# jmloveyj/ros_navigation

Measured on AMD Instinct MI355X. Metric: replan cycles/sec (HIMM+VFH++A*) on 4096x4096 grid, higher is better.
Workload: dtype int32; 1 GPU; full replan loop on 4096x4096 f32 grid (res 0.05 m); one step = one turn of the 20-stage A* pipeline = 20 passes of [100032-ray HIMM batch + fused compose -> 256 VFH+ poses -> 256 grid-A* queries (one launch)]; 30% rectangle obstacles (seed 2); 4 ray batches / pose sets / query sets in rotation; cycles_per_pass=256, rays_per_pass=100032, rotating_input_sets=4, astar_queries_checked=15360, astar_queries_answered=15360, astar_bucket_width=128000, astar_pipeline_depth=20, parallelism=query-sharded x1, full=False

## Files before the change

### ros_navigation_amd/csrc/astar_tile.hip

```cpp
#include "engine.hpp"
#include <algorithm>
#include <cstring>
#include <vector>

using namespace rna;

namespace rna {

constexpr int TI = 64, TJ = 16;
constexpr int TILE_WORDS = TI * TJ;
constexpr int AUX_WORDS = 64;
constexpr int MASK_STRIDE = TILE_WORDS + 32 + 128;
#ifndef RNA_TSA_WAVES
#define RNA_TSA_WAVES 8
#endif
#ifndef RNA_TSA_SUPER
#define RNA_TSA_SUPER 2
#endif
#ifndef RNA_TSA_HPASS
#define RNA_TSA_HPASS (RNA_TSA_SUPER == 2 ? 4 : (RNA_TSA_SUPER ? 8 : 16))
#endif
#ifndef RNA_TSA_FRESH
#define RNA_TSA_FRESH 0
#endif
#ifndef RNA_TSA_CONFIRM
#define RNA_TSA_CONFIRM 0
#endif
#ifndef RNA_TSA_IDLE_SLEEP
#define RNA_TSA_IDLE_SLEEP 4
#endif
#ifndef RNA_TSA_FIRST_ROWS
#define RNA_TSA_FIRST_ROWS 1
#endif
#ifndef RNA_TSA_REDBLACK
#define RNA_TSA_REDBLACK 1
#endif
#ifndef RNA_TSA_WAVES_PER_EU
#define RNA_TSA_WAVES_PER_EU 8
#endif
constexpr int TSA_WAVES = RNA_TSA_WAVES;
constexpr int TSA_MAX_TILE_WORDS = 2048;
constexpr int COST_S = 1000, COST_D = 1414;
constexpr int INF = 0x7fffffff;
constexpr int KU = 0x40000000;
constexpr int SCR_CNT = 84 + 192 + 48 + 64;
constexpr int SCR_WORDS = SCR_CNT + 4;
static_assert(SCR_WORDS % 4 == 0 && 276 % 4 == 0, "a wavefront's scratch starts on 16 bytes and so do the edge columns in it (ds_write_b128)");

__device__ __forceinline__ int tsa_octile(int i, int j, int gi, int gj) {
  const int dx = abs(i - gi), dy = abs(j - gj);
  const int mx = dx > dy ? dx : dy, mn = dx > dy ? dy : dx;
  return COST_S * mx + (COST_D - COST_S) * mn;
}
#ifndef RNA_TSA_SCOPE
#define RNA_TSA_SCOPE __HIP_MEMORY_SCOPE_AGENT
#endif
__device__ __forceinline__ unsigned ld_l2(const unsigned* p) {
  return __hip_atomic_load(p, __ATOMIC_RELAXED, RNA_TSA_SCOPE);
}
__device__ __forceinline__ int tsa_unwrap_lin(int lin, int rows, int cols, int s0, int s1) {
  int i = lin % rows - s0, j = lin / rows - s1;
  if (i < 0) i += rows;
  if (j < 0) j += cols;
  return j * rows + i;
}
__device__ __forceinline__ int tsa_buffer_lin(int lin, int rows, int cols, int s0, int s1) {
  int i = lin % rows + s0, j = lin / rows + s1;
  if (i >= rows) i -= rows;
  if (j >= cols) j -= cols;
  return j * rows + i;
}
__device__ __forceinline__ int lane_m1(int v) { return __builtin_amdgcn_update_dpp(0, v, 0x138, 0xF, 0xF, true); }
__device__ __forceinline__ int lane_p1(int v) { return __builtin_amdgcn_update_dpp(0, v, 0x130, 0xF, 0xF, true); }
// ... 27 lines not shown
#define TSA_OPEN(m, bit) ({ int r_; asm volatile("v_bfe_i32 %0, %1, %2, 1" : "=v"(r_) : "v"(m), "i"(bit)); r_; })
__device__ __forceinline__ int tsa_h24(int mx, int mn) {
  int a, r;
  asm("v_mul_u32_u24 %0, %2, %1" : "=v"(a) : "v"(mx), "s"(COST_S));
  asm("v_mad_u32_u24 %0, %1, %2, %3" : "=v"(r) : "v"(mn), "s"(COST_D - COST_S), "v"(a));
  return r;
}
__device__ __forceinline__ unsigned tsa_seed24(unsigned t, unsigned lane) {
  unsigned a, r;
  asm("v_mul_u32_u24 %0, %1, 29" : "=v"(a) : "v"(t));
  asm("v_mad_u32_u24 %0, %1, %2, %3" : "=v"(r) : "v"(lane), "s"(8191u), "v"(a));
  return r;
}
__device__ __forceinline__ int tsa_octile24(int i, int j, int gi, int gj) {
  const int dx = abs(i - gi), dy = abs(j - gj);
  return tsa_h24(max(dx, dy), min(dx, dy));
}
__device__ __forceinline__ int tsa_prop(int u, int h, int thr) { return (u - h >= thr) ? u : 0; }

__device__ __forceinline__ int tile_of(int i, int j, int tiles_i) { return (j >> 4) * tiles_i + (i >> 6); }
__device__ __forceinline__ int in_page(int i, int j) { return ((j & 15) << 6) + (i & 63); }
__device__ __forceinline__ int kdi_of(int k) { return (k == 0 || k == 3 || k == 5) ? -1 : ((k == 2 || k == 4 || k == 7) ? 1 : 0); }
__device__ __forceinline__ int kdj_of(int k) { return k < 3 ? -1 : (k > 4 ? 1 : 0); }

struct TsaStage {
  unsigned* pages;
  unsigned* paux;
  unsigned* tmap;
  unsigned* owner;
  int* nalloc;
  uint8_t* nbr_tm;
  int* perm;
  int* ticket;
  int cap;
};
__host__ __device__ inline size_t tsa_align256(size_t x) { return (x + 255) & ~(size_t)255; }
constexpr int TSA_COUNTER_WORDS = 16;
__host__ __device__ inline unsigned long long* tsa_counters_of(const TsaStage& S) {
  return reinterpret_cast<unsigned long long*>(reinterpret_cast<char*>(S.nalloc) - TSA_COUNTER_WORDS * sizeof(unsigned long long));
}

__global__ void __launch_bounds__(256) tsa_snapshot_kernel(const uint8_t* __restrict__ nbr, int rows, int cols, int tiles_i, int tiles_j,
                                                             uint8_t* __restrict__ nbr_tm, int s0, int s1) {
  __shared__ unsigned s_free[256];
  const int a = threadIdx.x & 63, bq = threadIdx.x >> 6;
  for (int t = blockIdx.x; t < tiles_i * tiles_j; t += gridDim.x) {
    const int i = (t % tiles_i) * TI + a, j0 = (t / tiles_i) * TJ + bq * 4;
    unsigned v = 0u;
    if (i < rows) {
      const int bi = i + s0 >= rows ? i + s0 - rows : i + s0;
#pragma unroll
      for (int k = 0; k < 4; ++k)
        if (j0 + k < cols) {
          const int bj = j0 + k + s1 >= cols ? j0 + k + s1 - cols : j0 + k + s1;
          v |= (unsigned)nbr[(size_t)bj * rows + bi] << (8 * k);
        }
    }
    uint8_t* out = nbr_tm + (size_t)t * MASK_STRIDE;
    reinterpret_cast<unsigned*>(out)[a * 4 + bq] = v;
    if (a == 0) reinterpret_cast<unsigned*>(out + TILE_WORDS)[bq] = v;
    if (a == TI - 1) reinterpret_cast<unsigned*>(out + TILE_WORDS + 16)[bq] = v;
    s_free[threadIdx.x] = (((v & 0xffu) != 0u) ? 1u : 0u) | (((v & 0xff00u) != 0u) ? 2u : 0u) | (((v & 0xff0000u) != 0u) ? 4u : 0u) |
                          (((v & 0xff000000u) != 0u) ? 8u : 0u);
    __syncthreads();
    if (bq == 0)
      reinterpret_cast<unsigned short*>(out + TILE_WORDS + 32)[a] =
// ... 772 lines not shown
  TSA_T(t_d);
  TSA_ACC(2, t_c, t_d);
  TSA_ACC(6, t_w0, t_d);
  if (lane_in == 0) { atomicAdd(&scr[SCR_CNT], (unsigned)__builtin_popcount(rowchg)); atomicAdd(&scr[SCR_CNT + 1], 1u); }
  }
tsa_job_done:
#ifndef RNA_TSA_UNSAFE_NOWAIT
  asm volatile("s_waitcnt vmcnt(0)" ::: "memory");
#endif
  {
    int t_f = t_in;
    asm volatile("" : "+s"(t_f));
    const int again = sch.finish(t_f, lane_in, spare, scr + SCR_CNT);
    if (!again) break;
    first_w = again >> 1;
    sticky_w = 1;
    TSA_CNT(7, 1);
    TSA_CNT(22, 1);
  }
  }
#undef TSA_ROW_CHANGED
#undef TSA_H
}

#ifndef RNA_TSA_NODES
#define RNA_TSA_NODES 3072
#endif
constexpr int TSA_NP = RNA_TSA_NODES;
constexpr int TSA_BMW = TSA_NP / 32;
#ifndef RNA_TSA_QC
#define RNA_TSA_QC 1024
#endif
constexpr int TSA_QC = RNA_TSA_QC;
constexpr unsigned POP_EMPTY = 0xffffffffu;
static_assert(TSA_NP % 32 == 0 && TSA_NP < 0xffff, "node indices are 16 bits, 0xffff = none");
static_assert(TSA_NP * 4 >= (TI + 2) * (TJ + 2) * 4 + TILE_WORDS, "the backtrace's LDS image lives in the queue memory");

__device__ __forceinline__ unsigned lds_ld(const unsigned* p) { return __hip_atomic_load(p, __ATOMIC_RELAXED, __HIP_MEMORY_SCOPE_WORKGROUP); }
__device__ __forceinline__ int lds_ldi(const int* p) { return __hip_atomic_load(p, __ATOMIC_RELAXED, __HIP_MEMORY_SCOPE_WORKGROUP); }

struct TsaLocalSched {
  int* best_;
  int* state_;
  unsigned* st2_;
  unsigned* far_;
  unsigned* node_;
  unsigned* head_;
  unsigned* bm_;
  unsigned* qc_;
  int* count_;
  int* spill_;
  unsigned* open_;
  int* open_left_;
  __device__ __forceinline__ int best() const { return __hip_atomic_load(best_, __ATOMIC_RELAXED, __HIP_MEMORY_SCOPE_WORKGROUP); }
  __device__ __forceinline__ void improve_best(int g) { atomicMin(best_, g); }
  __device__ __forceinline__ void overflow() { *state_ = 4; }
  __device__ __forceinline__ void pool_exhausted() { *state_ = 5; }
  __device__ __forceinline__ void act_far(int t) { atomicOr(&far_[t >> 5], 1u << (t & 31)); }
  __device__ __forceinline__ bool is_far(int t) const { return (lds_ld(&far_[t >> 5]) >> (t & 31)) & 1u; }
  __device__ __forceinline__ int node_alloc(unsigned seed) {
    unsigned w = ((seed & 0xffffu) * (unsigned)TSA_BMW) >> 16;
    for (int tries = 0; tries < 32; ++tries) {
      const unsigned v = lds_ld(&bm_[w]);
      if (v) {
        const unsigned b = v & (0u - v);
        if (atomicAnd(&bm_[w], ~b) & b) return (int)(w * 32u) + __builtin_ctz(b);
      } else {
        w = w + 1u == (unsigned)TSA_BMW ? 0u : w + 1u;
      }
    }
    return -1;
  }
  __device__ __forceinline__ void node_free(int idx) { atomicOr(&bm_[idx >> 5], 1u << (idx & 31)); }
  __device__ __forceinline__ void link(int idx, unsigned t, unsigned cls) {
    for (;;) {
      const unsigned hv = lds_ld(&head_[cls]);
      __hip_atomic_store(&node_[idx], (hv << 16) | t, __ATOMIC_RELAXED, __HIP_MEMORY_SCOPE_WORKGROUP);
      asm volatile("" ::: "memory");
      if (atomicCAS(&head_[cls], hv, ((hv + 0x10000u) & 0xffff0000u) | (unsigned)idx) == hv) break;
    }
  }
  __device__ __forceinline__ void push(unsigned t, unsigned cls, int lane, int* spare) {
    if (lane == 0) {
      const int idx = *spare >= 0 ? *spare : node_alloc(t * 29u);
      if (idx >= 0) {
        link(idx, t, cls);
        atomicAdd(count_, 1);
        __hip_atomic_store(&qc_[t & (unsigned)(TSA_QC - 1)], (t << 8) | cls, __ATOMIC_RELAXED, __HIP_MEMORY_SCOPE_WORKGROUP);
      } else {
        atomicOr(&far_[t >> 5], 1u << (t & 31));
        *spill_ = 1;
      }
    }
    *spare = -1;
  }
  __device__ __forceinline__ void wake8(bool w, int t, unsigned cls, int lane, int* spare) {
    const unsigned sh = 2u * ((unsigned)t & 15u);
    unsigned old = 2u;
    if (w) old = atomicOr(&st2_[t >> 4], 1u << sh) >> sh;
    bool q = w && !(old & 2u);
    const unsigned qi = (unsigned)t & (unsigned)(TSA_QC - 1);
    if (q && (old & 1u)) {
      const unsigned c = lds_ld(&qc_[qi]);
      if ((c >> 8) == (unsigned)t && (c & 0xffu) <= cls) q = false;
    }
    if (q) __hip_atomic_store(&qc_[qi], ((unsigned)t << 8) | cls, __ATOMIC_RELAXED, __HIP_MEMORY_SCOPE_WORKGROUP);
    const unsigned long long qm = __builtin_amdgcn_ballot_w64(q);
    if (!qm) return;
    const int reuse = *spare;
    *spare = -1;
    int idx = -1;
    if (q) {
      idx = (reuse >= 0 && lane == __builtin_ctzll(qm)) ? reuse : node_alloc(tsa_seed24((unsigned)t, (unsigned)lane));
      if (idx >= 0) {
        link(idx, (unsigned)t, cls);
      } else {
        atomicOr(&far_[t >> 5], 1u << (t & 31));
        *spill_ = 1;
      }
    }
    const unsigned long long okm = __builtin_amdgcn_ballot_w64(idx >= 0);
    if (okm && lane == __builtin_ctzll(okm)) atomicAdd(count_, __builtin_popcountll(okm));
  }
  __device__ __forceinline__ int finish(int t, int lane, int* spare, unsigned* cnt) {
    const unsigned sh = 2u * ((unsigned)t & 15u);
    int r = 0;
    if (lane == 0) {
      atomicAdd(&cnt[2], 1u);
#ifdef RNA_TSA_NO_STICKY
      if (false) {
#else
      if ((lds_ld(&st2_[t >> 4]) >> sh) & 1u) {
#endif
        atomicAnd(&st2_[t >> 4], ~(1u << sh));
// ... 139 lines not shown
      const unsigned mc = s_mask[il * 16 + jl];
      const unsigned un = s_tile[(jl + 1) * BW + il + 1 + off];
      const bool hit = (lane < 8) & (((mc >> k) & 1u) != 0u) & (un != 0u) & (un == uc + (unsigned)wk);
      const unsigned long long m = __ballot(hit);
      if (!m) { ok = false; break; }
      const int src = __builtin_ctz((unsigned)m);
      uc = (unsigned)__builtin_amdgcn_readlane((int)un, src);
      const int sdi = kdi_of(src), sdj = kdj_of(src);
      ci += sdi; cj += sdj; il += sdi; jl += sdj;
      if (il < 0 || jl < 0 || il >= TI || jl >= TJ) break;
    }
  }
#ifdef RNA_TSA_STATS
  if (lane == 0) { atomicAdd(&g_tsa_stat[27], bt_loads); atomicAdd(&g_tsa_stat[28], bt_load_ticks); atomicAdd(&g_tsa_stat[29], (unsigned long long)len); }
#endif
  if (!ok) {
    if (lane == 0) A.results[q] = rna_astar_result{1, 0, INF, r.expanded, r.rounds, r.buckets};
    return;
  }
  if (len > A.max_path_len || len > A.rev_cap) {
    if (lane == 0) A.results[q] = rna_astar_result{3, len, r.cost, r.expanded, r.rounds, r.buckets};
    return;
  }
  asm volatile("s_waitcnt vmcnt(0)" ::: "memory");
  __builtin_amdgcn_wave_barrier();
  int32_t* path = A.paths + (size_t)q * A.max_path_len;
  for (int i = lane; i < len; i += 64) path[i] = tsa_buffer_lin(rev[len - 1 - i], rows, cols, A.s0, A.s1);
  if (lane == 0) A.results[q] = rna_astar_result{0, len, r.cost, r.expanded, r.rounds, r.buckets};
}

template <int WAVES, bool RETRY>
__global__ void __launch_bounds__(WAVES * 64) __attribute__((amdgpu_waves_per_eu(RNA_TSA_WAVES_PER_EU, RNA_TSA_WAVES_PER_EU))) tsa_search_kernel(const TsaLaunch A) {
  constexpr int TSA_THREADS = WAVES * 64;
  __shared__ __attribute__((aligned(16))) unsigned s_scr[WAVES][SCR_WORDS];
  extern __shared__ unsigned s_dyn[];
  __shared__ __attribute__((aligned(16))) unsigned s_node[TSA_NP];
  __shared__ __attribute__((aligned(16))) unsigned s_head[TSA_NCLS];
  __shared__ unsigned s_bm[TSA_BMW];
  __shared__ unsigned s_qc[TSA_QC];
  __shared__ int s_best, s_state, s_bucket, s_bucket0, s_jobs_done, s_jobs_noop, s_jobs_sticky, s_expanded, s_nalloc, s_any;
  __shared__ int s_count, s_spill, s_idle, s_open_left, s_open_pos, s_reruns;

  __shared__ int s_q, s_rank;
  if (!RETRY) {
    if (threadIdx.x == 0) { const int k = atomicAdd(A.S.ticket, 1); s_rank = k; s_q = A.S.perm[k]; }
  } else {
    if (threadIdx.x == 0) { s_q = A.retry_list[A.retry_base + (int)blockIdx.x]; s_rank = 1 << 30; }
  }
  __syncthreads();
  const int q = __builtin_amdgcn_readfirstlane(s_q);
  if (q < 0) return;
  if (RETRY && threadIdx.x == 0) A.S2.ticket[8 + blockIdx.x] = q;
  const TsaStage& S = RETRY ? A.S2 : A.S;
  const int sl = RETRY ? (int)blockIdx.x : q;
#ifndef RNA_TSA_PRIO_FIRST
#define RNA_TSA_PRIO_FIRST 0
#endif
  if (__builtin_amdgcn_readfirstlane(s_rank) < A.prio_first) __builtin_amdgcn_s_setprio(3);
  const int tid = threadIdx.x, lane = tid & 63, wv = __builtin_amdgcn_readfirstlane(tid >> 6);
#ifdef RNA_TSA_STATS
  const unsigned long long t_kernel0 = wall_clock64();
#endif
  const int rows = A.rows, cols = A.cols, tiles_i = A.tiles_i, tiles_j = A.tiles_j;
  rna_astar_query qu = A.queries[q];
  const int ncell = rows * cols;
  const int ntile = tiles_i * tiles_j;
  const int nt_words = (ntile + 31) >> 5;
  unsigned* const s_st2 = s_dyn;
  unsigned* const s_open = s_dyn + 2 * nt_words;
  unsigned* const s_far = s_dyn + 3 * nt_words;
  rna_astar_result* const results = A.results;

  const bool valid = qu.start >= 0 && qu.goal >= 0 && qu.start < ncell && qu.goal < ncell;
  if (!valid) {
    if (tid == 0) results[q] = rna_astar_result{2, 0, INF, 0, 0, 0};
    return;
  }
  qu.start = tsa_unwrap_lin(qu.start, rows, cols, A.s0, A.s1);
  qu.goal = tsa_unwrap_lin(qu.goal, rows, cols, A.s0, A.s1);
  const int si = qu.start % rows, sj = qu.start / rows;
  const int gi = qu.goal % rows, gj = qu.goal / rows;

  TsaCtx C;
  C.rows = rows; C.cols = cols; C.tiles_i = tiles_i; C.tiles_j = tiles_j;
  C.tiles_magic = tiles_i > 1 ? (unsigned)(0x100000000ull / (unsigned)tiles_i) + 1u : 0u;
  C.pages = S.pages + (((size_t)sl * ((size_t)S.cap + 1)) << 10);
  C.paux = S.paux + (size_t)sl * ((size_t)S.cap + 1) * AUX_WORDS;
  C.tmap = S.tmap + (size_t)sl * ntile;
  C.owner = S.owner + (size_t)sl * (S.cap + 1);
  C.cap = S.cap;
  C.nalloc = &s_nalloc;
  C.nbr_tm = S.nbr_tm;
  C.gi = gi; C.gj = gj;
  C.ts = tile_of(si, sj, tiles_i); C.sa = si & (TI - 1); C.sb = sj & (TJ - 1);
  C.tg = tile_of(gi, gj, tiles_i); C.ga = gi & (TI - 1); C.gb = gj & (TJ - 1);

  for (int w = tid; w < 4 * nt_words; w += TSA_THREADS) s_dyn[w] = 0u;
  for (int w = tid; w < TSA_NCLS; w += TSA_THREADS) s_head[w] = 0xffffu;
  for (int w = tid; w < TSA_BMW; w += TSA_THREADS) s_bm[w] = 0xffffffffu;
  for (int w = tid; w < TSA_QC; w += TSA_THREADS) s_qc[w] = 0xffffffffu;
  if (lane >= 48) s_scr[wv][68 + lane - 48] = 0u;
  if (lane < 4) s_scr[wv][SCR_CNT + lane] = 0u;
  {
    const unsigned ms = C.nbr_tm[(size_t)C.ts * MASK_STRIDE + C.sa * 16 + C.sb], mg = C.nbr_tm[(size_t)C.tg * MASK_STRIDE + C.ga * 16 + C.gb];
    if (qu.goal != qu.start && (mg == 0u || ms == 0u)) {
      if (tid == 0) results[q] = rna_astar_result{1, 0, INF, 0, 0, 0};
      return;
    }
  }
  {
    const int used_raw = S.nalloc[sl];
    const int used = used_raw < C.cap ? used_raw : C.cap;
    if (used > 0) {
      uint4* pg4 = reinterpret_cast<uint4*>(C.pages + (1 << 10));
      for (size_t w = tid; w < (size_t)used * (TILE_WORDS / 4); w += TSA_THREADS) pg4[w] = make_uint4(0u, 0u, 0u, 0u);
      uint4* ax4 = reinterpret_cast<uint4*>(C.paux + AUX_WORDS);
      for (size_t w = tid; w < (size_t)used * (AUX_WORDS / 4); w += TSA_THREADS) ax4[w] = make_uint4(0u, 0u, 0u, 0u);
      for (int p = 1 + tid; p <= used; p += TSA_THREADS) C.tmap[C.owner[p]] = 0u;
      asm volatile("s_waitcnt vmcnt(0)" ::: "memory");
    }
  }
  int key_shift = 0;
  while (((long long)A.bucket_width >> key_shift) > TSA_NCLS - 1) ++key_shift;
  if (tid == 0) {
    s_best = INF; s_state = 0; s_jobs_done = 0; s_jobs_noop = 0; s_jobs_sticky = 0; s_expanded = 0; s_nalloc = 0;
    s_bucket = tsa_octile(si, sj, gi, gj) / A.bucket_width;
    s_bucket0 = s_bucket;
    s_spill = 0; s_idle = 0; s_open_pos = 0; s_reruns = 0;
    s_count = 1; s_open_left = 1;
  }
  __syncthreads();
  if (tid == 0) s_open[C.ts >> 5] = 1u << (C.ts & 31);
  __syncthreads();

#ifdef RNA_TSA_STATS
  unsigned long long tsa_acc[24] = {};
  const unsigned long long t_life0 = wall_clock64();
  const unsigned long long c_life0 = __builtin_amdgcn_s_memtime();
#endif
#ifdef RNA_TSA_IDLE
  unsigned long long idle_ticks = 0ull;
  const unsigned long long t_wave0 = __builtin_amdgcn_s_memtime();
#endif
  TsaLocalSched sch{&s_best, &s_state, s_st2, s_far, s_node, s_head, s_bm, s_qc, &s_count, &s_spill, s_open, &s_open_left};
  int spare = -1;

  for (;;) {
    const int bucket = __builtin_amdgcn_readfirstlane(lds_ldi(&s_bucket));
    const long long bucket_end = ((long long)bucket + 1) * A.bucket_width;
    const unsigned bucket_end_u = bucket_end > 0x80000000LL ? 0x80000000u : (unsigned)bucket_end;
    const long long key_base_ll = (long long)KU - (long long)bucket * A.bucket_width;
    const int key_base = key_base_ll < -(long long)INF ? -INF : (int)key_base_ll;
    bool idle = false;
    bool open_blocked = false;
#ifdef RNA_TSA_IDLE
    unsigned long long t_idle0 = 0ull;
#endif
    for (;;) {
      TSA_T(t_p0);
      if (lds_ldi(&s_state) >= 4) break;
      if (idle) {
        if (lds_ldi(&s_idle) == WAVES) break;
        if (lds_ldi(&s_count) <= 0) { __builtin_amdgcn_s_sleep(RNA_TSA_IDLE_SLEEP); continue; }
        if (lane == 0) atomicSub(&s_idle, 1);
        idle = false;
#ifdef RNA_TSA_IDLE
        idle_ticks += __builtin_amdgcn_s_memtime() - t_idle0;
#endif
      }
      int t = -1;
      int first = 0;
      const int open_left = lds_ldi(&s_open_left);
      if (!open_blocked && open_left > 0) {
        const int pos = lds_ldi(&s_open_pos);
        const unsigned w = pos + lane < nt_words ? lds_ld(&s_open[pos + lane]) : 0u;
        const unsigned long long nz = __builtin_amdgcn_ballot_w64(w != 0u);
        if (!nz) {
          if (lane == 0) atomicCAS(&s_open_pos, pos, pos + 64 >= nt_words ? 0 : pos + 64);
          continue;
        }
        const int l0 = __builtin_ctzll(nz);
        const unsigned w0 = (unsigned)__builtin_amdgcn_readlane((int)w, l0);
        const int b0 = __builtin_ctz(w0);
        const int tt = ((pos + l0) << 5) + b0;
        const unsigned sh = 2u * ((unsigned)tt & 15u);
        int r = 0;
        if (lane == 0) {
          if ((atomicAnd(&s_open[pos + l0], ~(1u << b0)) >> b0) & 1u) {
            const unsigned old = atomicOr(&s_st2[tt >> 4], 2u << sh) >> sh;
            if (old & 2u) {
              atomicOr(&s_open[pos + l0], 1u << b0);
              atomicOr(&s_st2[tt >> 4], 1u << sh);
              r = 2;
            } else {
              atomicAnd(&s_st2[tt >> 4], ~(1u << sh));
              atomicSub(&s_open_left, 1);
              atomicSub(&s_count, 1);
              r = 1;
            }
          }
        }
        r = __builtin_amdgcn_readfirstlane(r);
        if (r == 0) continue;
        if (r == 2) { open_blocked = true; continue; }
        t = tt;
        first = 1;
      } else {
        open_blocked = false;
        const unsigned e = sch.pop(lane, &spare);
        if (e == POP_EMPTY) {
          if (open_left > 0) { __builtin_amdgcn_s_sleep(2); continue; }
          if (lane == 0) atomicAdd(&s_idle, 1);
          idle = true;
#ifdef RNA_TSA_IDLE
          t_idle0 = __builtin_amdgcn_s_memtime();
#endif
          continue;
        }
        const int tt = (int)(e & 0xffffu);
        const unsigned sh = 2u * ((unsigned)tt & 15u);
        int r = 0;
        if (lane == 0) {
          unsigned w = lds_ld(&s_st2[tt >> 4]);
          while (((w >> sh) & 3u) == 1u) {
            const unsigned got = atomicCAS(&s_st2[tt >> 4], w, (w | (2u << sh)) & ~(1u << sh));
            if (got == w) { r = 1; break; }
            w = got;
          }
          if (r == 1 && open_left > 0 && ((atomicAnd(&s_open[tt >> 5], ~(1u << (tt & 31))) >> (tt & 31)) & 1u)) {
            atomicSub(&s_open_left, 1);
            atomicSub(&s_count, 1);
            r = 2;
          }
        }
        r = __builtin_amdgcn_readfirstlane(r);
        if (r <= 0) continue;
        t = tt;
        first = r >> 1;
      }
#ifdef RNA_TSA_TAKE_SLEEP
      __builtin_amdgcn_s_sleep(RNA_TSA_TAKE_SLEEP);
#endif
      TSA_T(t_p1);
      TSA_ACC(4, t_p0, t_p1);
      TSA_CNT(7, 1);
#if defined(RNA_TSA_JOBPRIO)
      __builtin_amdgcn_s_setprio(RNA_TSA_JOBPRIO);
#endif
      tsa_job(sch, s_scr[wv], lane, t, C, first, bucket_end_u, key_base, key_shift, &spare TSA_ACC_ARG);
#if defined(RNA_TSA_JOBPRIO)
      __builtin_amdgcn_s_setprio(RNA_TSA_IDLEPRIO);
#endif
    }
    __syncthreads();
#ifdef RNA_TSA_IDLE
    if (idle) idle_ticks += __builtin_amdgcn_s_memtime() - t_idle0;
#endif
    if (s_state >= 4) break;
    int tid_r = threadIdx.x;
    asm volatile("" : "+v"(tid_r));
    const bool spilled = s_spill != 0;
    __syncthreads();
    if (tid_r == 0) {
      if (!spilled && s_best != INF && (long long)s_best < bucket_end) s_state = 1;
      if (spilled) s_reruns += 1;
      s_any = 0; s_spill = 0; s_idle = 0; s_open_pos = 0;
    }
    __syncthreads();
    if (s_state == 1) break;
    int cnt = 0;
    for (int w = tid_r; w < nt_words; w += TSA_THREADS) {
      const unsigned b = s_far[w];
      s_open[w] = b;
      s_far[w] = 0u;
      cnt += __popc(b);
    }
    if (cnt) atomicAdd(&s_any, cnt);
    __syncthreads();
    if (tid_r == 0) {
      if (!s_any) s_state = (s_best != INF) ? 1 : 2;
      else { s_count = s_any; s_open_left = s_any; if (!spilled) s_bucket += 1; }
    }
    __syncthreads();
    if (s_state != 0) break;
  }
#ifdef RNA_TSA_IDLE
  if (lane == 0) {
    atomicAdd(&tsa_counters_of(S)[8], __builtin_amdgcn_s_memtime() - t_wave0);
    atomicAdd(&tsa_counters_of(S)[9], idle_ticks);
  }
#endif
  if (lane == 0) {
    atomicAdd(&s_expanded, (int)s_scr[wv][SCR_CNT] * TI);
    atomicAdd(&s_jobs_done, (int)s_scr[wv][SCR_CNT + 2]);
    atomicAdd(&s_jobs_noop, (int)(s_scr[wv][SCR_CNT + 2] - s_scr[wv][SCR_CNT + 1]));
    atomicAdd(&s_jobs_sticky, (int)s_scr[wv][SCR_CNT + 3]);
  }
  __syncthreads();
  if (tid == 0) {
    unsigned long long* const cnt = tsa_counters_of(S);
    atomicAdd(&cnt[0], 1ull);
    atomicAdd(&cnt[1], (unsigned long long)s_nalloc);
    atomicAdd(&cnt[2], (unsigned long long)s_jobs_done);
    atomicAdd(&cnt[3], (unsigned long long)s_jobs_noop);
    atomicAdd(&cnt[4], (unsigned long long)s_jobs_sticky);
    atomicAdd(&cnt[5], (unsigned long long)(s_expanded / TI));
    atomicAdd(&cnt[6], (unsigned long long)(s_bucket - s_bucket0 + 1));
    if (s_reruns) atomicAdd(&cnt[7], (unsigned long long)s_reruns);
  }
#ifdef RNA_TSA_STATS
// ... 41 lines not shown
    for (int r = 0; r < TSA_RETRY; ++r)
      if (served[r] == q) { sl = r; retried = true; }
  if (!retried)
    for (int r = 0; r < n_retried; ++r)
      if (retry_list[r] == q) { if (threadIdx.x == 0) counts[q] = -1; return; }
  const TsaStage& S = retried ? S_retry : S_main;
  if (threadIdx.x == 0) s_cnt = 0;
  __syncthreads();
  const rna_astar_result r = results[q];
  int cnt = 0;
  if (r.status == 0 || r.status == 3) {
    const int goal = tsa_unwrap_lin(queries[q].goal, rows, cols, s0, s1);
    const int gi = goal % rows, gj = goal / rows;
    const int used = S.nalloc[sl];
    for (size_t w = threadIdx.x; w < ((size_t)used << 10); w += blockDim.x) {
      const int p = 1 + (int)(w >> 10), l = (int)(w & 1023);
      const int t = (int)S.owner[(size_t)sl * (S.cap + 1) + p];
      const int i = (t % tiles_i) * TI + (l & (TI - 1)), j = (t / tiles_i) * TJ + (l >> 6);
      const unsigned u = S.pages[(((size_t)sl * ((size_t)S.cap + 1) + p) << 10) + l];
      if (u != 0u && i < rows && j < cols && (KU - (int)u) + tsa_octile(i, j, gi, gj) <= r.cost) ++cnt;
    }
  }
  atomicAdd(&s_cnt, cnt);
  __syncthreads();
  if (threadIdx.x == 0) counts[q] = s_cnt;
}

static inline int tsa_ntile(const rna_engine* e) {
  return ((e->geom.size[0] + TI - 1) / TI) * ((e->geom.size[1] + TJ - 1) / TJ);
}
bool tsa_supported(const rna_engine* e) { return (size_t)tsa_ntile(e) <= (size_t)TSA_MAX_TILE_WORDS * 32; }
int tsa_tiles(const rna_engine* e) { return tsa_ntile(e); }
size_t tsa_pool_bytes(int max_queries, int cap) { return (size_t)max_queries * ((size_t)cap + 1) * (TILE_WORDS + AUX_WORDS) * sizeof(unsigned); }
size_t tsa_aux_bytes(const rna_engine* e, int max_queries, int cap) {
  const size_t ntile = (size_t)tsa_ntile(e);
  return 256 + 2 * tsa_align256((size_t)max_queries * sizeof(int)) + tsa_align256(ntile * MASK_STRIDE) +
         tsa_align256((size_t)max_queries * ntile * sizeof(unsigned)) + tsa_align256((size_t)max_queries * ((size_t)cap + 1) * sizeof(unsigned));
}
static TsaStage tsa_stage_view(const rna_engine* e, int slot) {
  const AstarDevice& a = e->astar;
  const size_t ntile = (size_t)tsa_ntile(e);
  char* base = static_cast<char*>(a.tsa_aux[slot]);
  TsaStage S;
  S.cap = a.page_cap;
  S.pages = reinterpret_cast<unsigned*>(a.g[slot]);
  S.paux = S.pages + (((size_t)a.max_queries * ((size_t)S.cap + 1)) << 10);
  S.ticket = reinterpret_cast<int*>(base);
  base += 256;
  S.nalloc = reinterpret_cast<int*>(base);
  base += tsa_align256((size_t)a.max_queries * sizeof(int));
  S.perm = reinterpret_cast<int*>(base);
  base += tsa_align256((size_t)a.max_queries * sizeof(int));
  S.nbr_tm = reinterpret_cast<uint8_t*>(base);
  base += tsa_align256(ntile * MASK_STRIDE);
  S.tmap = reinterpret_cast<unsigned*>(base);
  base += tsa_align256((size_t)a.max_queries * ntile * sizeof(unsigned));
  S.owner = reinterpret_cast<unsigned*>(base);
  return S;
}
size_t tsa_retry_pool_bytes(const rna_engine* e) { return tsa_pool_bytes(TSA_RETRY, tsa_ntile(e)); }
size_t tsa_retry_aux_bytes(const rna_engine* e) {
  const size_t ntile = (size_t)tsa_ntile(e);
  return 256 + tsa_align256(TSA_RETRY * sizeof(int)) + tsa_align256((size_t)TSA_RETRY * ntile * sizeof(unsigned)) +
         tsa_align256((size_t)TSA_RETRY * (ntile + 1) * sizeof(unsigned)) + tsa_align256((size_t)e->astar.max_queries * sizeof(int));
}
static int* tsa_retry_list(const rna_engine* e, int slot) {
  const size_t ntile = (size_t)tsa_ntile(e);
  return reinterpret_cast<int*>(static_cast<char*>(e->astar.tsa_aux_retry[slot]) + 256 + tsa_align256(TSA_RETRY * sizeof(int)) +
                                tsa_align256((size_t)TSA_RETRY * ntile * sizeof(unsigned)) + tsa_align256((size_t)TSA_RETRY * (ntile + 1) * sizeof(unsigned)));
}
static int* tsa_retry_served(const rna_engine* e, int slot) { return reinterpret_cast<int*>(e->astar.tsa_aux_retry[slot]) + 8; }
static int* tsa_retry_count(const rna_engine* e, int slot) { return tsa_retry_served(e, slot) + TSA_RETRY; }
static TsaStage tsa_retry_view(const rna_engine* e, int slot, const TsaStage& main) {
  const AstarDevice& a = e->astar;
  const size_t ntile = (size_t)tsa_ntile(e);
  char* base = static_cast<char*>(a.tsa_aux_retry[slot]);
  TsaStage S = main;
  S.cap = (int)ntile;
  S.pages = reinterpret_cast<unsigned*>(a.g_retry[slot]);
  S.paux = S.pages + (((size_t)TSA_RETRY * ((size_t)S.cap + 1)) << 10);
  S.ticket = reinterpret_cast<int*>(base);
  base += 256;
  S.nalloc = reinterpret_cast<int*>(base);
  base += tsa_align256(TSA_RETRY * sizeof(int));
  S.tmap = reinterpret_cast<unsigned*>(base);
  base += tsa_align256((size_t)TSA_RETRY * ntile * sizeof(unsigned));
  S.owner = reinterpret_cast<unsigned*>(base);
  return S;
}
int tsa_retry_prepare(rna_engine* e, int slot) {
  hipLaunchKernelGGL(tsa_fill_pages_kernel, dim3(2048), dim3(256), 0, e->stream, reinterpret_cast<uint4*>(e->astar.g_retry[slot]),
                     tsa_retry_pool_bytes(e) / sizeof(uint4));
  RNA_HIP(e, hipGetLastError());
  return RNA_OK;
}
int tsa_stage_prepare(rna_engine* e, int slot) {
  const TsaStage S = tsa_stage_view(e, slot);
  const size_t pages = (size_t)e->astar.max_queries * ((size_t)S.cap + 1);
  hipLaunchKernelGGL(tsa_fill_pages_kernel, dim3(8192), dim3(256), 0, e->stream, reinterpret_cast<uint4*>(S.pages),
                     pages * (TILE_WORDS + AUX_WORDS) / 4);
  RNA_HIP(e, hipGetLastError());
  return RNA_OK;
}

size_t tsa_ring_bytes(const rna_engine* e, int max_queries) {
  return 256 + tsa_align256((size_t)max_queries * sizeof(int)) + tsa_align256((size_t)tsa_ntile(e) * MASK_STRIDE);
}
static_assert(sizeof(TsaLaunch) <= sizeof(AstarDevice::last_launch[0]), "AstarDevice::last_launch holds a TsaLaunch");

int tsa_retry_launch(rna_engine* e, int slot, hipStream_t search_stream, int count) {
  AstarDevice& a = e->astar;
  TsaLaunch A;
  memcpy(&A, a.last_launch[slot], sizeof(A));
  A.retry = 1;
  A.retry_count = nullptr;
  A.S2 = tsa_retry_view(e, slot, A.S);
  for (int base = 0; base < count; base += TSA_RETRY) {
    A.retry_base = base;
    const int wgs = std::min(TSA_RETRY, count - base);
    if (a.depth > 1) hipLaunchKernelGGL((tsa_search_kernel<TSA_WAVES, true>), dim3(wgs), dim3(TSA_WAVES * 64), a.last_lds[slot], search_stream, A);
    else hipLaunchKernelGGL((tsa_search_kernel<16, true>), dim3(wgs), dim3(16 * 64), a.last_lds[slot], search_stream, A);
    RNA_HIP(e, hipGetLastError());
  }
  return RNA_OK;
}

int tsa_launch(rna_engine* e, int slot, hipStream_t init_stream, hipStream_t search_stream, hipEvent_t ev_init,
               const rna_astar_query* q_dev, int n, int32_t* paths_dev, int max_len, rna_astar_result* res_dev) {
  AstarDevice& a = e->astar;
  const int rows = e->geom.size[0], cols = e->geom.size[1];
  const int ti = (rows + TI - 1) / TI, tj = (cols + TJ - 1) / TJ;
  TsaStage S = tsa_stage_view(e, slot);
  hipStream_t prep_stream = search_stream;
  int ring = -1;
  if (ev_init) {
    ring = (int)(a.launches % (unsigned long long)a.ring_n);
    char* base = a.ring_mem + (size_t)ring * a.ring_stride;
    S.ticket = reinterpret_cast<int*>(base);
    S.perm = reinterpret_cast<int*>(base + 256);
    S.nbr_tm = reinterpret_cast<uint8_t*>(base + 256 + tsa_align256((size_t)a.max_queries * sizeof(int)));
    { const int rc = side_stream(e, &prep_stream); if (rc != RNA_OK) return rc; }
    RNA_HIP(e, hipEventRecord(ev_init, init_stream));
    RNA_HIP(e, hipStreamWaitEvent(prep_stream, ev_init, 0));
    if (a.ring_used[ring]) RNA_HIP(e, hipStreamWaitEvent(prep_stream, a.ring_free[ring], 0));
  }
  {
    KernelTimer kt(e, RNA_K_ASTAR_INIT, prep_stream);
    hipLaunchKernelGGL(tsa_snapshot_kernel, dim3(std::min(ti * tj, 4096)), dim3(256), 0, prep_stream, e->nbr, rows, cols, ti, tj, S.nbr_tm,
                       e->geom.start[0], e->geom.start[1]);
    RNA_HIP(e, hipGetLastError());
  }
  if (ev_init) {
    RNA_HIP(e, hipEventRecord(a.snap_done[slot], prep_stream));
    a.snap_pending[slot] = true;
  }
  {
    KernelTimer kt(e, RNA_K_ASTAR_RESET, prep_stream);
    const int ranked = n <= 2048 ? 1 : 0;
    hipLaunchKernelGGL(tsa_prepare_kernel, dim3(1), dim3(256), ranked ? (size_t)n * sizeof(int) : 0, prep_stream, S, q_dev, n, rows, cols, ranked,
                       a.g_retry[slot] ? tsa_retry_served(e, slot) : nullptr);
    RNA_HIP(e, hipGetLastError());
  }
  if (ev_init) {
    RNA_HIP(e, hipEventRecord(a.ev_prep, prep_stream));
    RNA_HIP(e, hipStreamWaitEvent(search_stream, a.ev_prep, 0));
  }
  {
    KernelTimer kt(e, RNA_K_ASTAR_SEARCH, search_stream);
    const size_t nt_bytes = (size_t)((ti * tj + 31) / 32) * sizeof(unsigned);
    TsaLaunch A;
    memset(&A, 0, sizeof(A));
    A.rows = rows; A.cols = cols; A.tiles_i = ti; A.tiles_j = tj; A.s0 = e->geom.start[0]; A.s1 = e->geom.start[1];
    A.queries = q_dev; A.S = S; A.bucket_width = a.bucket_width; A.paths = paths_dev; A.max_path_len = max_len;
    A.rev_all = a.rev[slot]; A.rev_cap = a.rev_cap; A.results = res_dev;
    A.retry = 0; A.n = n; A.S2 = S;
    A.prio_first = a.depth > 1 ? RNA_TSA_PRIO_FIRST : 0;
    if (const char* pf = getenv("RNA_TSA_PRIO_FIRST")) A.prio_first = atoi(pf);
    size_t lds_dyn = 4 * nt_bytes;
    if (const char* pad = getenv("RNA_TSA_LDS_PAD")) lds_dyn += (size_t)atoi(pad);
    const bool can_retry = a.g_retry[slot] != nullptr && a.retry_flag != nullptr;
    A.retry_count = can_retry ? tsa_retry_count(e, slot) : nullptr;
    A.retry_list = can_retry ? tsa_retry_list(e, slot) : nullptr;
    A.retry_base = 0;
    if (can_retry) a.retry_flag[slot] = 0;
    a.last_retried[slot] = 0;
    static const bool wide_env = getenv("RNA_TSA_WIDE") != nullptr;
    const bool wide = wide_env || n <= 32;
    if (a.depth > 1 && !wide) hipLaunchKernelGGL((tsa_search_kernel<TSA_WAVES, false>), dim3(n), dim3(TSA_WAVES * 64), lds_dyn, search_stream, A);
    else hipLaunchKernelGGL((tsa_search_kernel<16, false>), dim3(n), dim3(16 * 64), lds_dyn, search_stream, A);
    RNA_HIP(e, hipGetLastError());
    memcpy(a.last_launch[slot], &A, sizeof(A));
    a.last_lds[slot] = lds_dyn;
    a.retry_armed[slot] = A.retry_count != nullptr;
    if (A.retry_count) RNA_HIP(e, hipMemcpyAsync(a.retry_flag + slot, A.retry_count, sizeof(int), hipMemcpyDeviceToHost, search_stream));
  }
  if (ring >= 0) {
    RNA_HIP(e, hipEventRecord(a.ring_free[ring], search_stream));
    a.ring_used[ring] = true;
  }
  return RNA_OK;
}

int tsa_counters_read(rna_engine* e, unsigned long long* out, bool reset) {
  AstarDevice& a = e->astar;
  for (int k = 0; k < TSA_COUNTER_WORDS; ++k) out[k] = 0ull;
  for (int d = 0; d < AstarDevice::MAX_DEPTH; ++d) {
    for (int view = 0; view < 2; ++view) {
      char* base = static_cast<char*>(view ? a.tsa_aux_retry[d] : a.tsa_aux[d]);
      if (!base) continue;
      unsigned long long w[TSA_COUNTER_WORDS];
      char* cnt = base + 256 - sizeof(w);
      RNA_HIP(e, hipMemcpyAsync(w, cnt, sizeof(w), hipMemcpyDeviceToHost, e->stream));
      if (reset) RNA_HIP(e, hipMemsetAsync(cnt, 0, sizeof(w), e->stream));
      RNA_HIP(e, hipStreamSynchronize(e->stream));
      for (int k = 0; k < TSA_COUNTER_WORDS; ++k) out[k] += w[k];
    }
  }
  return RNA_OK;
}

#ifdef RNA_TSA_STATS
void tsa_stats_dump() {
  unsigned long long st[32];
  if (hipMemcpyFromSymbol(st, HIP_SYMBOL(g_tsa_stat), sizeof(st)) != hipSuccess) return;
  const double jobs = (double)st[7];
// ... 38 lines not shown
```

### ros_navigation_amd/csrc/engine.hpp

```cpp
#pragma once

#include <hip/hip_runtime.h>

#include <cstdint>
#include <cstdio>
#include <string>
#include <vector>

#include "../../include/rna.h"
#include "gridmath.hpp"

namespace rna {

constexpr int TILE = 64;

struct HimmSlot { int cell; int head; int len; int offset; };

struct HimmScratch {
  int cap_rays = 0;
  int n_slots = 0;
  rna_ray* rays_dev = nullptr;
  int4* desc = nullptr;
  int* ncells = nullptr;
  int* next = nullptr;
// ... 37 lines not shown
#ifndef RNA_ASTAR_MAX_DEPTH
#define RNA_ASTAR_MAX_DEPTH 20
#endif
  static constexpr int MAX_DEPTH = RNA_ASTAR_MAX_DEPTH;
  int depth = 4;
  int32_t* g[MAX_DEPTH] = {};
  int2* queues[MAX_DEPTH] = {};
  int32_t* rev[MAX_DEPTH] = {};
  int rev_cap = 16800;
  int mode = 1;
  int page_cap = 0;
  int page_cap_request = 0;
  void* tsa_aux[MAX_DEPTH] = {};
  int32_t* g_retry[MAX_DEPTH] = {};
  void* tsa_aux_retry[MAX_DEPTH] = {};
  hipStream_t side[MAX_DEPTH] = {};
  hipEvent_t done[MAX_DEPTH] = {};
  hipEvent_t snap_done[MAX_DEPTH] = {};
  bool snap_pending[MAX_DEPTH] = {};
  bool busy[MAX_DEPTH] = {};
  unsigned long long stage_seq[MAX_DEPTH] = {};
  hipEvent_t ev_init = nullptr;
  static constexpr int MAX_RING = 2 * MAX_DEPTH;
  int ring_n = 0;
  char* ring_mem = nullptr;
  size_t ring_stride = 0;
  hipEvent_t ring_free[MAX_RING] = {};
  bool ring_used[MAX_RING] = {};
  hipEvent_t ev_prep = nullptr;
  int* retry_flag = nullptr;
  bool retry_armed[MAX_DEPTH] = {};
  int last_retried[MAX_DEPTH] = {};
  size_t last_lds[MAX_DEPTH] = {};
  alignas(8) unsigned char last_launch[MAX_DEPTH][384] = {};
  unsigned long long launches = 0;
  int last_slot = 0;
  size_t field_stride = 0;
  rna_astar_query* queries_dev = nullptr;
  rna_astar_result* results_dev = nullptr;
  int32_t* paths_dev = nullptr;
  int paths_cap = 0;
  const rna_astar_query* last_queries = nullptr;
  const rna_astar_result* last_results = nullptr;
  int last_n = 0;
};

struct FootprintPlan {
  double r = 0.0, res = 0.0, mag = 0.0;
  int R = 0;
  int K = 0;
  int band = 0;
  int n_ties = 0;
  int w[64] = {};
};

struct ProfSlot {
  double total_ms = 0;
  int64_t launches = 0;
  std::vector<std::pair<hipEvent_t, hipEvent_t>> pending;
};

}

struct rna_engine {
  rna::Geom geom{};
  int device = 0;
// ... 124 lines not shown
```

Measured before the change: 164,100 replan cycles/s.

## Move open/far tile bitmaps from LDS to global and allow 4-wave search kernel

Moves the per-query open and far tile bitsets out of dynamic LDS into a per-slot global buffer that is accessed with agent-scope atomics, which halves the dynamic LDS footprint. Templates the local scheduler on the queue-cache size so that a 4-wave variant can use a smaller LDS cache. Adds a runtime env selection between 4 and 8 waves and records the chosen width for retry launches. The aim is lower LDS usage per workgroup and higher occupancy, at the cost of global-memory latency and extra atomics on the bitmap operations in the hot scheduling loop.

```diff
diff --git a/ros_navigation_amd/csrc/astar_tile.hip b/ros_navigation_amd/csrc/astar_tile.hip
--- a/ros_navigation_amd/csrc/astar_tile.hip
+++ b/ros_navigation_amd/csrc/astar_tile.hip
@@ -39,6 +39,7 @@
 #define RNA_TSA_WAVES_PER_EU 8
 #endif
 constexpr int TSA_WAVES = RNA_TSA_WAVES;
+static_assert(TSA_WAVES == 4 || TSA_WAVES == 8, "the pipelined search kernel is instantiated for 4 and 8 wavefronts");
 constexpr int TSA_MAX_TILE_WORDS = 2048;
 constexpr int COST_S = 1000, COST_D = 1414;
 constexpr int INF = 0x7fffffff;
@@ -132,6 +133,7 @@
   uint8_t* nbr_tm;
   int* perm;
   int* ticket;
+  unsigned* tbits;
   int cap;
 };
 __host__ __device__ inline size_t tsa_align256(size_t x) { return (x + 255) & ~(size_t)255; }
@@ -970,6 +972,7 @@
 #define RNA_TSA_QC 1024
 #endif
 constexpr int TSA_QC = RNA_TSA_QC;
+constexpr int TSA_QC_NARROW = 256;
 constexpr unsigned POP_EMPTY = 0xffffffffu;
 static_assert(TSA_NP % 32 == 0 && TSA_NP < 0xffff, "node indices are 16 bits, 0xffff = none");
 static_assert(TSA_NP * 4 >= (TI + 2) * (TJ + 2) * 4 + TILE_WORDS, "the backtrace's LDS image lives in the queue memory");
@@ -977,6 +980,7 @@
 __device__ __forceinline__ unsigned lds_ld(const unsigned* p) { return __hip_atomic_load(p, __ATOMIC_RELAXED, __HIP_MEMORY_SCOPE_WORKGROUP); }
 __device__ __forceinline__ int lds_ldi(const int* p) { return __hip_atomic_load(p, __ATOMIC_RELAXED, __HIP_MEMORY_SCOPE_WORKGROUP); }
 
+template <int QC>
 struct TsaLocalSched {
   int* best_;
   int* state_;
@@ -995,7 +999,7 @@
   __device__ __forceinline__ void overflow() { *state_ = 4; }
   __device__ __forceinline__ void pool_exhausted() { *state_ = 5; }
   __device__ __forceinline__ void act_far(int t) { atomicOr(&far_[t >> 5], 1u << (t & 31)); }
-  __device__ __forceinline__ bool is_far(int t) const { return (lds_ld(&far_[t >> 5]) >> (t & 31)) & 1u; }
+  __device__ __forceinline__ bool is_far(int t) const { return (ld_l2(&far_[t >> 5]) >> (t & 31)) & 1u; }
   __device__ __forceinline__ int node_alloc(unsigned seed) {
     unsigned w = ((seed & 0xffffu) * (unsigned)TSA_BMW) >> 16;
     for (int tries = 0; tries < 32; ++tries) {
@@ -1024,7 +1028,7 @@
       if (idx >= 0) {
         link(idx, t, cls);
         atomicAdd(count_, 1);
-        __hip_atomic_store(&qc_[t & (unsigned)(TSA_QC - 1)], (t << 8) | cls, __ATOMIC_RELAXED, __HIP_MEMORY_SCOPE_WORKGROUP);
+        __hip_atomic_store(&qc_[t & (unsigned)(QC - 1)], (t << 8) | cls, __ATOMIC_RELAXED, __HIP_MEMORY_SCOPE_WORKGROUP);
       } else {
         atomicOr(&far_[t >> 5], 1u << (t & 31));
         *spill_ = 1;
@@ -1037,7 +1041,7 @@
     unsigned old = 2u;
     if (w) old = atomicOr(&st2_[t >> 4], 1u << sh) >> sh;
     bool q = w && !(old & 2u);
-    const unsigned qi = (unsigned)t & (unsigned)(TSA_QC - 1);
+    const unsigned qi = (unsigned)t & (unsigned)(QC - 1);
     if (q && (old & 1u)) {
       const unsigned c = lds_ld(&qc_[qi]);
       if ((c >> 8) == (unsigned)t && (c & 0xffu) <= cls) q = false;
@@ -1243,12 +1247,13 @@
 template <int WAVES, bool RETRY>
 __global__ void __launch_bounds__(WAVES * 64) __attribute__((amdgpu_waves_per_eu(RNA_TSA_WAVES_PER_EU, RNA_TSA_WAVES_PER_EU))) tsa_search_kernel(const TsaLaunch A) {
   constexpr int TSA_THREADS = WAVES * 64;
+  constexpr int QC = WAVES == 4 ? TSA_QC_NARROW : TSA_QC;
   __shared__ __attribute__((aligned(16))) unsigned s_scr[WAVES][SCR_WORDS];
   extern __shared__ unsigned s_dyn[];
   __shared__ __attribute__((aligned(16))) unsigned s_node[TSA_NP];
   __shared__ __attribute__((aligned(16))) unsigned s_head[TSA_NCLS];
   __shared__ unsigned s_bm[TSA_BMW];
-  __shared__ unsigned s_qc[TSA_QC];
+  __shared__ unsigned s_qc[QC];
   __shared__ int s_best, s_state, s_bucket, s_bucket0, s_jobs_done, s_jobs_noop, s_jobs_sticky, s_expanded, s_nalloc, s_any;
   __shared__ int s_count, s_spill, s_idle, s_open_left, s_open_pos, s_reruns;
 
@@ -1278,8 +1283,8 @@
   const int ntile = tiles_i * tiles_j;
   const int nt_words = (ntile + 31) >> 5;
   unsigned* const s_st2 = s_dyn;
-  unsigned* const s_open = s_dyn + 2 * nt_words;
-  unsigned* const s_far = s_dyn + 3 * nt_words;
+  unsigned* const g_open = S.tbits + (size_t)sl * 2 * nt_words;
+  unsigned* const g_far = g_open + nt_words;
   rna_astar_result* const results = A.results;
 
   const bool valid = qu.start >= 0 && qu.goal >= 0 && qu.start < ncell && qu.goal < ncell;
@@ -1306,10 +1311,10 @@
   C.ts = tile_of(si, sj, tiles_i); C.sa = si & (TI - 1); C.sb = sj & (TJ - 1);
   C.tg = tile_of(gi, gj, tiles_i); C.ga = gi & (TI - 1); C.gb = gj & (TJ - 1);
 
-  for (int w = tid; w < 4 * nt_words; w += TSA_THREADS) s_dyn[w] = 0u;
+  for (int w = tid; w < 2 * nt_words; w += TSA_THREADS) s_dyn[w] = 0u;
   for (int w = tid; w < TSA_NCLS; w += TSA_THREADS) s_head[w] = 0xffffu;
   for (int w = tid; w < TSA_BMW; w += TSA_THREADS) s_bm[w] = 0xffffffffu;
-  for (int w = tid; w < TSA_QC; w += TSA_THREADS) s_qc[w] = 0xffffffffu;
+  for (int w = tid; w < QC; w += TSA_THREADS) s_qc[w] = 0xffffffffu;
   if (lane >= 48) s_scr[wv][68 + lane - 48] = 0u;
   if (lane < 4) s_scr[wv][SCR_CNT + lane] = 0u;
   {
@@ -1320,6 +1325,7 @@
     }
   }
   {
+    for (int w = tid; w < 2 * nt_words; w += TSA_THREADS) g_open[w] = 0u;
     const int used_raw = S.nalloc[sl];
     const int used = used_raw < C.cap ? used_raw : C.cap;
     if (used > 0) {
@@ -1328,8 +1334,8 @@
       uint4* ax4 = reinterpret_cast<uint4*>(C.paux + AUX_WORDS);
       for (size_t w = tid; w < (size_t)used * (AUX_WORDS / 4); w += TSA_THREADS) ax4[w] = make_uint4(0u, 0u, 0u, 0u);
       for (int p = 1 + tid; p <= used; p += TSA_THREADS) C.tmap[C.owner[p]] = 0u;
-      asm volatile("s_waitcnt vmcnt(0)" ::: "memory");
-    }
+    }
+    asm volatile("s_waitcnt vmcnt(0)" ::: "memory");
   }
   int key_shift = 0;
   while (((long long)A.bucket_width >> key_shift) > TSA_NCLS - 1) ++key_shift;
@@ -1341,7 +1347,10 @@
     s_count = 1; s_open_left = 1;
   }
   __syncthreads();
-  if (tid == 0) s_open[C.ts >> 5] = 1u << (C.ts & 31);
+  if (tid == 0) {
+    atomicOr(&g_open[C.ts >> 5], 1u << (C.ts & 31));
+    asm volatile("s_waitcnt vmcnt(0)" ::: "memory");
+  }
   __syncthreads();
 
 #ifdef RNA_TSA_STATS
@@ -1353,7 +1362,7 @@
   unsigned long long idle_ticks = 0ull;
   const unsigned long long t_wave0 = __builtin_amdgcn_s_memtime();
 #endif
-  TsaLocalSched sch{&s_best, &s_state, s_st2, s_far, s_node, s_head, s_bm, s_qc, &s_count, &s_spill, s_open, &s_open_left};
+  TsaLocalSched<QC> sch{&s_best, &s_state, s_st2, g_far, s_node, s_head, s_bm, s_qc, &s_count, &s_spill, g_open, &s_open_left};
   int spare = -1;
 
   for (;;) {
@@ -1384,7 +1393,7 @@
       const int open_left = lds_ldi(&s_open_left);
       if (!open_blocked && open_left > 0) {
         const int pos = lds_ldi(&s_open_pos);
-        const unsigned w = pos + lane < nt_words ? lds_ld(&s_open[pos + lane]) : 0u;
+        const unsigned w = pos + lane < nt_words ? ld_l2(&g_open[pos + lane]) : 0u;
         const unsigned long long nz = __builtin_amdgcn_ballot_w64(w != 0u);
         if (!nz) {
           if (lane == 0) atomicCAS(&s_open_pos, pos, pos + 64 >= nt_words ? 0 : pos + 64);
@@ -1397,10 +1406,10 @@
         const unsigned sh = 2u * ((unsigned)tt & 15u);
         int r = 0;
         if (lane == 0) {
-          if ((atomicAnd(&s_open[pos + l0], ~(1u << b0)) >> b0) & 1u) {
+          if ((atomicAnd(&g_open[pos + l0], ~(1u << b0)) >> b0) & 1u) {
             const unsigned old = atomicOr(&s_st2[tt >> 4], 2u << sh) >> sh;
             if (old & 2u) {
-              atomicOr(&s_open[pos + l0], 1u << b0);
+              atomicOr(&g_open[pos + l0], 1u << b0);
               atomicOr(&s_st2[tt >> 4], 1u << sh);
               r = 2;
             } else {
@@ -1438,7 +1447,7 @@
             if (got == w) { r = 1; break; }
             w = got;
           }
-          if (r == 1 && open_left > 0 && ((atomicAnd(&s_open[tt >> 5], ~(1u << (tt & 31))) >> (tt & 31)) & 1u)) {
+          if (r == 1 && open_left > 0 && ((atomicAnd(&g_open[tt >> 5], ~(1u << (tt & 31))) >> (tt & 31)) & 1u)) {
             atomicSub(&s_open_left, 1);
             atomicSub(&s_count, 1);
             r = 2;
@@ -1481,12 +1490,13 @@
     if (s_state == 1) break;
     int cnt = 0;
     for (int w = tid_r; w < nt_words; w += TSA_THREADS) {
-      const unsigned b = s_far[w];
-      s_open[w] = b;
-      s_far[w] = 0u;
+      const unsigned b = ld_l2(&g_far[w]);
+      g_open[w] = b;
+      g_far[w] = 0u;
       cnt += __popc(b);
     }
     if (cnt) atomicAdd(&s_any, cnt);
+    asm volatile("s_waitcnt vmcnt(0)" ::: "memory");
     __syncthreads();
     if (tid_r == 0) {
       if (!s_any) s_state = (s_best != INF) ? 1 : 2;
@@ -1594,10 +1604,14 @@
 bool tsa_supported(const rna_engine* e) { return (size_t)tsa_ntile(e) <= (size_t)TSA_MAX_TILE_WORDS * 32; }
 int tsa_tiles(const rna_engine* e) { return tsa_ntile(e); }
 size_t tsa_pool_bytes(int max_queries, int cap) { return (size_t)max_queries * ((size_t)cap + 1) * (TILE_WORDS + AUX_WORDS) * sizeof(unsigned); }
+static size_t tsa_tbits_bytes(const rna_engine* e, int slots) {
+  return tsa_align256((size_t)slots * 2 * (((size_t)tsa_ntile(e) + 31) / 32) * sizeof(unsigned));
+}
 size_t tsa_aux_bytes(const rna_engine* e, int max_queries, int cap) {
   const size_t ntile = (size_t)tsa_ntile(e);
   return 256 + 2 * tsa_align256((size_t)max_queries * sizeof(int)) + tsa_align256(ntile * MASK_STRIDE) +
-         tsa_align256((size_t)max_queries * ntile * sizeof(unsigned)) + tsa_align256((size_t)max_queries * ((size_t)cap + 1) * sizeof(unsigned));
+         tsa_align256((size_t)max_queries * ntile * sizeof(unsigned)) + tsa_align256((size_t)max_queries * ((size_t)cap + 1) * sizeof(unsigned)) +
+         tsa_tbits_bytes(e, max_queries);
 }
 static TsaStage tsa_stage_view(const rna_engine* e, int slot) {
   const AstarDevice& a = e->astar;
@@ -1618,13 +1632,16 @@
   S.tmap = reinterpret_cast<unsigned*>(base);
   base += tsa_align256((size_t)a.max_queries * ntile * sizeof(unsigned));
   S.owner = reinterpret_cast<unsigned*>(base);
+  base += tsa_align256((size_t)a.max_queries * ((size_t)S.cap + 1) * sizeof(unsigned));
+  S.tbits = reinterpret_cast<unsigned*>(base);
   return S;
 }
 size_t tsa_retry_pool_bytes(const rna_engine* e) { return tsa_pool_bytes(TSA_RETRY, tsa_ntile(e)); }
 size_t tsa_retry_aux_bytes(const rna_engine* e) {
   const size_t ntile = (size_t)tsa_ntile(e);
   return 256 + tsa_align256(TSA_RETRY * sizeof(int)) + tsa_align256((size_t)TSA_RETRY * ntile * sizeof(unsigned)) +
-         tsa_align256((size_t)TSA_RETRY * (ntile + 1) * sizeof(unsigned)) + tsa_align256((size_t)e->astar.max_queries * sizeof(int));
+         tsa_align256((size_t)TSA_RETRY * (ntile + 1) * sizeof(unsigned)) + tsa_align256((size_t)e->astar.max_queries * sizeof(int)) +
+         tsa_tbits_bytes(e, TSA_RETRY);
 }
 static int* tsa_retry_list(const rna_engine* e, int slot) {
   const size_t ntile = (size_t)tsa_ntile(e);
@@ -1648,6 +1665,7 @@
   S.tmap = reinterpret_cast<unsigned*>(base);
   base += tsa_align256((size_t)TSA_RETRY * ntile * sizeof(unsigned));
   S.owner = reinterpret_cast<unsigned*>(base);
+  S.tbits = reinterpret_cast<unsigned*>(reinterpret_cast<char*>(tsa_retry_list(e, slot)) + tsa_align256((size_t)a.max_queries * sizeof(int)));
   return S;
 }
 int tsa_retry_prepare(rna_engine* e, int slot) {
@@ -1669,6 +1687,20 @@
   return 256 + tsa_align256((size_t)max_queries * sizeof(int)) + tsa_align256((size_t)tsa_ntile(e) * MASK_STRIDE);
 }
 static_assert(sizeof(TsaLaunch) <= sizeof(AstarDevice::last_launch[0]), "AstarDevice::last_launch holds a TsaLaunch");
+
+static int tsa_pipelined_waves() {
+  if (const char* w = getenv("RNA_TSA_WAVES")) {
+    const int v = atoi(w);
+    if (v == 4 || v == 8) return v;
+  }
+  return TSA_WAVES;
+}
+template <bool RETRY>
+static void tsa_launch_search(int waves, int wgs, size_t lds_dyn, hipStream_t stream, const TsaLaunch& A) {
+  if (waves == 4) hipLaunchKernelGGL((tsa_search_kernel<4, RETRY>), dim3(wgs), dim3(4 * 64), lds_dyn, stream, A);
+  else if (waves == 8) hipLaunchKernelGGL((tsa_search_kernel<8, RETRY>), dim3(wgs), dim3(8 * 64), lds_dyn, stream, A);
+  else hipLaunchKernelGGL((tsa_search_kernel<16, RETRY>), dim3(wgs), dim3(16 * 64), lds_dyn, stream, A);
+}
 
 int tsa_retry_launch(rna_engine* e, int slot, hipStream_t search_stream, int count) {
   AstarDevice& a = e->astar;
@@ -1680,8 +1712,7 @@
   for (int base = 0; base < count; base += TSA_RETRY) {
     A.retry_base = base;
     const int wgs = std::min(TSA_RETRY, count - base);
-    if (a.depth > 1) hipLaunchKernelGGL((tsa_search_kernel<TSA_WAVES, true>), dim3(wgs), dim3(TSA_WAVES * 64), a.last_lds[slot], search_stream, A);
-    else hipLaunchKernelGGL((tsa_search_kernel<16, true>), dim3(wgs), dim3(16 * 64), a.last_lds[slot], search_stream, A);
+    tsa_launch_search<true>(a.last_waves[slot], wgs, a.last_lds[slot], search_stream, A);
     RNA_HIP(e, hipGetLastError());
   }
   return RNA_OK;
@@ -1738,7 +1769,7 @@
     A.retry = 0; A.n = n; A.S2 = S;
     A.prio_first = a.depth > 1 ? RNA_TSA_PRIO_FIRST : 0;
     if (const char* pf = getenv("RNA_TSA_PRIO_FIRST")) A.prio_first = atoi(pf);
-    size_t lds_dyn = 4 * nt_bytes;
+    size_t lds_dyn = 2 * nt_bytes;
     if (const char* pad = getenv("RNA_TSA_LDS_PAD")) lds_dyn += (size_t)atoi(pad);
     const bool can_retry = a.g_retry[slot] != nullptr && a.retry_flag != nullptr;
     A.retry_count = can_retry ? tsa_retry_count(e, slot) : nullptr;
@@ -1748,11 +1779,12 @@
     a.last_retried[slot] = 0;
     static const bool wide_env = getenv("RNA_TSA_WIDE") != nullptr;
     const bool wide = wide_env || n <= 32;
-    if (a.depth > 1 && !wide) hipLaunchKernelGGL((tsa_search_kernel<TSA_WAVES, false>), dim3(n), dim3(TSA_WAVES * 64), lds_dyn, search_stream, A);
-    else hipLaunchKernelGGL((tsa_search_kernel<16, false>), dim3(n), dim3(16 * 64), lds_dyn, search_stream, A);
+    const int waves = a.depth > 1 && !wide ? tsa_pipelined_waves() : 16;
+    tsa_launch_search<false>(waves, n, lds_dyn, search_stream, A);
     RNA_HIP(e, hipGetLastError());
     memcpy(a.last_launch[slot], &A, sizeof(A));
     a.last_lds[slot] = lds_dyn;
+    a.last_waves[slot] = waves;
     a.retry_armed[slot] = A.retry_count != nullptr;
     if (A.retry_count) RNA_HIP(e, hipMemcpyAsync(a.retry_flag + slot, A.retry_count, sizeof(int), hipMemcpyDeviceToHost, search_stream));
   }
diff --git a/ros_navigation_amd/csrc/engine.hpp b/ros_navigation_amd/csrc/engine.hpp
--- a/ros_navigation_amd/csrc/engine.hpp
+++ b/ros_navigation_amd/csrc/engine.hpp
@@ -93,6 +93,7 @@
   bool retry_armed[MAX_DEPTH] = {};
   int last_retried[MAX_DEPTH] = {};
   size_t last_lds[MAX_DEPTH] = {};
+  int last_waves[MAX_DEPTH] = {};
   alignas(8) unsigned char last_launch[MAX_DEPTH][384] = {};
   unsigned long long launches = 0;
   int last_slot = 0;
```

New measurement: 163,600 replan cycles/s (median of 2 runs). About the same (-0.3%).
